# AsyncFlow-Sim/AsyncFlow

Measured on AMD Instinct MI355X. Metric: simulated request-events/sec (2-server LB scenario, 10k replicas/GPU), higher is better.
Workload: dtype f64

## Files before the change

### asyncflow_amd/csrc/af_core.hpp

```cpp
#pragma once

#include <stdint.h>

#include "af_math.hpp"

#if defined(__HIPCC__)
#define AF_CORE __device__ __forceinline__
#define AF_CORE_NOINLINE __device__ __noinline__
#define AF_PLAN_AS __attribute__((address_space(3)))
#else
#define AF_CORE inline
#define AF_CORE_NOINLINE __attribute__((noinline))
#define AF_PLAN_AS
#endif

namespace af {

enum : uint32_t { NODE_CLIENT = 0, NODE_LB = 1, NODE_SERVER = 2 };
enum : uint32_t { LB_ROUND_ROBIN = 0, LB_LEAST_CONNECTIONS = 1 };
enum : uint32_t { METRIC_READY = 1, METRIC_IO = 2, METRIC_RAM = 4, METRIC_EDGE = 8 };
enum : uint32_t {
    FLAG_POOL_OVERFLOW = 1u << 0,
    FLAG_FIFO_OVERFLOW = 1u << 1,
    FLAG_CLOCK_OVERFLOW = 1u << 2,
// ... 51 lines not shown
struct Layout {
    uint32_t cap;
    uint32_t fcap;
    uint32_t ovr_mask;
    uint32_t hk, ha, hb, edge, ring, stime, srv, cq, rq, lb, n_words;
    uint32_t srvram, marks;
    uint32_t tcap, tie_words;
};
#ifndef AF_RING_LOW
#define AF_RING_LOW 1
#endif
enum : uint32_t { LEDGE = 2, LSRV = 6, RING = 4, RING_LOW = AF_RING_LOW };

AF_HD Layout make_layout(uint32_t cap, uint32_t fcap, uint32_t n_edges, uint32_t n_servers, uint32_t n_lb,
                         uint32_t n_rows, uint32_t ovr_mask, uint32_t n_emarks = 0u, uint32_t n_smarks = 0u) {
    Layout L{};
    L.cap = cap;
    L.fcap = fcap;
    L.ovr_mask = ovr_mask;
    uint32_t w = 0;
    L.hk = w; w += cap;
    L.ha = w; w += cap;
    L.hb = w; w += cap;
    L.edge = w; w += LEDGE * n_edges;
    L.ring = w; w += RING * (1u + n_edges);
    L.stime = w; if (ovr_mask & (1u << PARAM_STEP_TIME)) w += n_rows;
    L.srv = w; w += LSRV * n_servers;
    L.cq = w; w += 2u * n_servers * fcap;
    L.rq = w; w += 2u * n_servers * fcap;
    L.lb = w; w += n_lb > 8u ? n_lb : 0u;
    L.srvram = w; if (ovr_mask & (1u << PARAM_SRV_RAM_MB)) w += n_servers;
    L.marks = w; if (ovr_mask & kParamMarkBits) w += 3u * n_emarks + 2u * n_smarks;
    L.n_words = w;
    uint32_t tc = 16u;
    while (tc < 2u * cap + 8u) tc <<= 1;
    L.tcap = tc;
    L.tie_words = 6u * tc + (2u + n_servers + 63u) / 64u + 17u;
    return L;
}
AF_HD uint64_t layout_bytes_per_lane(const Layout& L) { return 8ull * L.n_words; }

struct LaneOut {
    double* clock;
    uint32_t* samples;
    uint32_t* counts;
    uint32_t clock_cap, tick_cap, series_pitch;
    uint32_t* hist;
    uint32_t* rps;
    uint32_t hist_bins, rps_buckets;
    double hist_scale;
};

#if defined(__HIP_DEVICE_COMPILE__)
#define AF_BUMP(p) ((void)atomicAdd((p), 1u))
#else
#define AF_BUMP(p) ((void)(*(p) += 1u))
#endif

AF_HD void store4(uint32_t* p, uint32_t a, uint32_t b, uint32_t c, uint32_t d) {
#if defined(__HIP_DEVICE_COMPILE__)
    *reinterpret_cast<uint4*>(p) = make_uint4(a, b, c, d);
#else
    p[0] = a; p[1] = b; p[2] = c; p[3] = d;
#endif
}

constexpr double AF_INF = __builtin_huge_val();

struct PreDraws {
    const double* base;
    uint32_t n_per_stream;
    uint32_t flags_in;
    uint64_t* tie;
    AF_HD double entry(uint32_t stream, uint32_t index) const {
        return base[(size_t)stream * n_per_stream + index];
    }
};

AF_HD double pre_edge_draw(uint64_t seed, uint32_t e, uint32_t idx, uint32_t dist, double mean, double sigma,
                           double dropout) {
    const uint32_t stream = stream_edge(e);
    const U4 r = draw_block(seed, stream, idx, 0u);
    if (u53(r.x, r.y) < dropout) return -1.0;
    return test_quant(variate_from_u1(dist, mean, sigma, u53(r.z, r.w), seed, stream, idx));
}

struct GenState {
    double g_now = 0.0, g_wend = 0.0, g_lam = 0.0;
    uint32_t draws = 0;
};
AF_HD double gen_next_gap(GenState& g, uint64_t seed, uint32_t users_dist, double users_mean, double users_sigma,
                          double rpm, double window_s, double T) {
    const double rps_per_user = rpm / 60.0;
    while (g.g_now < T) {
        if (g.g_now >= g.g_wend) {
            g.g_wend = g.g_now + window_s;
            const uint32_t idx = g.draws++;
            double users;
            if (users_dist == DIST_NORMAL) {
                const double v = users_mean + users_sigma * af_norminv(uniform_j(seed, STREAM_GENERATOR, idx, 0u));
                users = v > 0.0 ? v : 0.0;
            } else {
                users = (double)af_poisson(users_mean, seed, STREAM_GENERATOR, idx, 0u);
            }
            g.g_lam = users * rps_per_user;
        }
        if (g.g_lam <= 0.0) {
            g.g_now = g.g_wend;
            continue;
        }
        const U4 r = draw_block(seed, STREAM_GENERATOR, g.draws++, 0u);
        double u = u53(r.x, r.y);
        if (u < 1e-15) u = 1e-15;
        const double dt = test_quant(-af_log_unit(1.0 - u) / g.g_lam);
        if (g.g_now + dt > T) break;
        if (g.g_now + dt >= g.g_wend) {
            g.g_now = g.g_wend;
            continue;
        }
        g.g_now += dt;
        return dt;
    }
    g.g_now = T + 1.0;
    return -1.0;
}

AF_CORE_NOINLINE uint32_t cold_endpoint_pick(uint64_t seed, uint32_t sv, uint32_t idx, uint32_t n_ep) {
    const U4 r = draw_block(seed, stream_server(sv), idx, 0u);
    return (uint32_t)(((uint64_t)r.x * n_ep) >> 32);
}

struct LaneRegs {
    double now, t_gen, t_tick, t_emark, t_smark;
    uint64_t lb_list;
    uint32_t q_gen, q_tick, q_emark, q_smark;
    uint32_t arr_ahead;
    int32_t dirty_edge;
    uint32_t fl;
    uint32_t heap_n, seq, live, max_live, lb_n, emark_i, smark_i;
    uint32_t n_gen, n_comp, n_drop, n_events, n_ticks, n_marks, flags;
    uint32_t pb_n;
};

template <bool kFaithful> struct RoundType { using type = uint32_t; };
template <> struct RoundType<false> { using type = bool; };

template <class Mem, bool kFaithful = true>
struct Lane : LaneRegs {
    const PlanView& P;
    const Layout& L;
    Mem M;
    LaneOut O;
    PreDraws D;
    uint64_t seed;

    enum : uint32_t {
        F_HOLE = 1u,
        F_GRANT = 2u,
        F_SEND = 4u,
        F_ADV = 8u,
        F_ADV_CORE = 16u,
        F_ADV_IO = 32u,
        F_DIRTY_ARR = 64u,
        F_SEND_FIRST = 128u
    };

    uint32_t pend_count;
// ... 1116 lines not shown
```

### asyncflow_amd/csrc/af_flow.hpp

```cpp
#pragma once

#include <stdint.h>

#include "af_core.hpp"

namespace aff {

using af::AF_INF;
using af::d2u;
using af::u2d;

enum : uint32_t {
    FLAG_FLOW_FALLBACK = 1u << 8,
    FLOW_WHY_TIE = 1u << 9,
    FLOW_WHY_LIST = 1u << 10,
    FLOW_WHY_RING = 1u << 11,
    FLOW_WHY_RAM = 1u << 12,
    FLOW_WHY_GEN_TIE = 1u << 15,
    FLOW_WHY_MASK = FLOW_WHY_TIE | FLOW_WHY_LIST | FLOW_WHY_RING | FLOW_WHY_RAM | FLOW_WHY_GEN_TIE,
};
constexpr uint32_t kMaxServers = 16;
constexpr uint32_t kSrvSlots = 16;
enum : uint32_t { LBW_ARRIVALS = 24u, LBW_SEG_OFF = LBW_ARRIVALS + kSrvSlots, LBW_SEG_LEN = LBW_SEG_OFF + kSrvSlots,
                  LBW_PROG = LBW_SEG_LEN + kSrvSlots, LBW_SLOTS = LBW_PROG + kSrvSlots, LBW_U32 = LBW_SLOTS + kSrvSlots };
// ... 365 lines not shown
                            if (u < n_left) {
                                if (!in_hbm) ring()[((r0 + u) & (R - 1u)) * pitch + ser] = 0;
                                value += d[u];
                                samples[(size_t)(r0 + u) * pitch + ser] = series_word(value, on, is_ram);
                            }
                    }
                }
            }
        }
        tick_base = upto;
    }

    AF_CORE double spike_at(uint32_t e, double now) {
        double sp = 0.0;
        if (A.n_edge_marks <= 32u) {
            for (uint32_t m = sends()[e]; m != 0u; m &= m - 1u) {
                const uint32_t i = (uint32_t)__builtin_ctz(m);
                const double tm = u2d(emark(i)[0]);
                if (tm < now) sp = spike_cum()[i];
                else if (tm == now) why |= FLOW_WHY_TIE;
            }
            return sp;
        }
        for (uint32_t i = 0u; i < A.n_edge_marks; ++i) {
            const double tm = u2d(emark(i)[0]);
            if ((uint32_t)emark(i)[2] != e) continue;
            if (tm < now) sp = spike_cum()[i];
            else if (tm == now) why |= FLOW_WHY_TIE;
        }
        return sp;
    }
    AF_CORE double send_floor(uint32_t st, double h, bool cached = true) {
        if (!(kMarks && A.n_edge_marks != 0u) || !(h < AF_INF)) return h;
        if (kLC && st == 2u) return h;
        AF_PLAN_AS double* c = fcache() + 3u * st;
        double until = c[0], sp_min = c[1], cand = c[2];
        if (!cached || !(h < until)) {
            until = cand = sp_min = AF_INF;
            const uint32_t n_out = st == 2u ? A.n_lb_edges : st == 3u ? A.n_servers : 1u;
            for (uint32_t k = 0u; k < n_out; ++k) {
                const uint32_t e = st == 0u   ? A.gen_out_edge
                                   : st == 1u ? A.client_out_edge
                                   : st == 2u ? (uint32_t)blob[A.off_lb + k]
                                              : (uint32_t)(blob[A.off_srv + af::SREC * k + 1u] >> 16) & 0xFFFFu;
                double sp = 0.0;
                for (uint32_t i = 0u; i < A.n_edge_marks; ++i) {
                    if ((uint32_t)emark(i)[2] != e) continue;
                    const double tm = u2d(emark(i)[0]), after = spike_cum()[i];
                    if (tm < h) {
                        sp = after;
                    } else {
                        until = tm < until ? tm : until;
                        cand = tm + after < cand ? tm + after : cand;
                    }
                }
                sp_min = sp < sp_min ? sp : sp_min;
            }
            if (cached && lane == 0u) {
                c[0] = until;
                c[1] = sp_min;
                c[2] = cand;
            }
        }
        const double fl = h + sp_min;
        return fl < cand ? fl : cand;
    }
    AF_CORE_NOINLINE static double cold_variate(uint32_t dist, double mean, double sigma, double u1, uint64_t seed, uint32_t stream,
                                                uint32_t idx) {
        return af::variate_from_u1(dist, mean, sigma, u1, seed, stream, idx);
    }
    AF_CORE bool edge_draw(uint32_t e, uint32_t idx, double& transit) const {
        const AF_PLAN_AS uint64_t* r = erec(e);
        const double mean = u2d(r[0]), sigma = u2d(r[1]);
        const uint32_t stream = af::stream_edge(e);
#if defined(__HIP_DEVICE_COMPILE__) && defined(AF_FJ_KEYS_PER_CALL)
        uint32_t sd_lo = (uint32_t)__builtin_amdgcn_readfirstlane((int)(uint32_t)seed), sd_hi = (uint32_t)__builtin_amdgcn_readfirstlane((int)(uint32_t)(seed >> 32));
        asm volatile("" : "+s"(sd_lo), "+s"(sd_hi));
        const af::U4 rr = af::draw_block(((uint64_t)sd_hi << 32) | sd_lo, stream, idx, 0u);
#else
        const af::U4 rr = af::draw_block(seed, stream, idx, 0u);
#endif
        const uint64_t k53 = ((uint64_t)(rr.x >> 5) << 26) | (uint64_t)(rr.y >> 6);
        const bool sent = !(k53 < r[2]);
        const double u1 = af::u53(rr.z, rr.w);
#if defined(AF_FJ_DIST_ALL) && (AF_FJ_DIST_ALL != 255)
        transit = af::test_quant(af::variate_from_u1(AF_FJ_DIST_ALL, mean, sigma, u1, seed, stream, idx));
#else
        const uint32_t dist = (uint32_t)(r[3] >> 16) & 0xFFu;
        transit = af::test_quant(dist == af::DIST_EXPONENTIAL ? -(mean * af::af_log_unit(1.0 - u1)) : cold_variate(dist, mean, sigma, u1, seed, stream, idx));
#endif
        return sent;
    }
    AF_CORE bool send_draw(uint32_t e, uint32_t idx, double& transit, bool pre = false, double pre_transit = 0.0) {
        transit = pre_transit;
        const bool sent = (kLC && pre) ? !(pre_transit < 0.0) : edge_draw(e, idx, transit);
        if (!sent) drops += 1u;
        return sent;
    }
    AF_CORE bool send_finish(uint32_t e, double now, uint32_t row_now, bool have_row, double transit, double& key, bool& counted) {
        counted = false;
        const double spike = (kMarks && A.n_edge_marks != 0u) ? spike_at(e, now) : 0.0;
        key = now + (transit + spike);
        if (transit + spike < 0.0) why |= FLOW_WHY_TIE;
        if (!kFar) {
            if (samples != nullptr) add_span(e, have_row ? row_now : tick_index(now, true), tick_index(key, true), 1);
        } else if (samples != nullptr) {
            const uint32_t ib = tick_index(key, true);
            if (ib != row_now) {
                add_point(e, row_now, 1);
                const uint32_t R = A.L.ring_rows, N = A.n_ticks < A.tick_cap ? A.n_ticks : A.tick_cap;
                if ((kHbmRing && R == 0u) || ib >= N || ib - tick_base < R) add_point(e, ib, -1);
                else counted = true;
            }
        }
        return true;
    }

    AF_CORE void append(uint32_t s, bool have, double key, double t0, uint32_t aux, double sent) {
        const uint64_t m = W::ballot(have);
        const uint32_t n = n_list_get(s);
        const uint32_t pos = n + W::mbcnt(m);
        if (have) {
            list_key(s)[pos] = key;
            list_t0(s)[pos] = t0;
            if (kTieBreak) list_ts(s)[pos] = sent;
            if (s == 2u || (kFar && s == 3u)) list_aux(s)[pos] = (uint16_t)aux;
        }
        n_list_set(s, n + popc64(m));
    }

    AF_CORE uint32_t select(uint32_t s, double H_in, uint32_t room, double& okey, double& ot0, uint32_t& oaux, uint32_t hs, uint32_t level = kAnyLevel) {
        if (kBig) return select_big(s, H_in, room, okey, ot0, oaux, hs, level);
        return select_regs<IPL>(s, H_in, room, okey, ot0, oaux, hs, level);
    }
    template <uint32_t IPLx>
    AF_CORE uint32_t select_regs(uint32_t s, double H_in, uint32_t room, double& okey, double& ot0, uint32_t& oaux, uint32_t hs, uint32_t level) {
        W::sync();
        const double lo = H_get(hs);
        const double hi_t = H_in < A.total_time ? H_in : A.total_time, hi = (kFar && t_lim < hi_t) ? t_lim : hi_t;
        const uint32_t n = n_list_get(s);
        okey = AF_INF;
        ot0 = 0.0;
        oaux = 0u;
        if (!(hi > lo)) return 0u;
        if (n == 0u) {
            H_set(hs, hi);
            return 0u;
        }
        AF_PLAN_AS double* K = list_key(s);
        AF_PLAN_AS double* T0 = list_t0(s);
        AF_PLAN_AS double* TS = list_ts(s);
        AF_PLAN_AS uint16_t* AX = list_aux(s);
        double sc = 64.0 * W::rcp(hi - lo);
        if (!(sc < 1e300)) sc = 1e300;
        hist()[lane] = 0u;
        W::sync();
        double k[IPLx], t[IPLx], sent[IPLx];
        uint32_t a[IPLx], b[IPLx], slot[IPLx];
        bool valid[IPLx], elig[IPLx];
#pragma unroll
        for (uint32_t q = 0u; q < IPLx; ++q) {
            valid[q] = elig[q] = false;
            k[q] = t[q] = sent[q] = 0.0;
            a[q] = b[q] = slot[q] = 0u;
            {
                const uint32_t i = q * 64u + lane;
                valid[q] = i < n;
                k[q] = K[i];
                t[q] = T0[i];
                if (kTieBreak) sent[q] = TS[i];
                a[q] = (s == 2u || (kFar && s == 3u)) ? AX[i] : 0u;
                elig[q] = valid[q] && k[q] < hi && (!kChain || level == kAnyLevel || level_of(a[q] & (kSrvSlots - 1u)) == level);
// ... 1813 lines not shown
```

### asyncflow_amd/csrc/af_math.hpp

```cpp
#pragma once

#include <stdint.h>

#if defined(__HIPCC__)
#define AF_HD __host__ __device__ __forceinline__
#else
#define AF_HD inline
#endif

namespace af {

constexpr uint32_t STREAM_GENERATOR = 0u;
AF_HD uint32_t stream_edge(uint32_t e) { return 1u + e; }
AF_HD uint32_t stream_server(uint32_t s) { return 0x1000u + s; }

struct U4 {
    uint32_t x, y, z, w;
};

AF_HD U4 philox4x32_10(uint32_t c0, uint32_t c1, uint32_t c2, uint32_t c3, uint32_t k0, uint32_t k1) {
#pragma unroll
    for (int r = 0; r < 10; ++r) {
        const uint64_t p0 = (uint64_t)0xD2511F53u * c0;
        const uint64_t p1 = (uint64_t)0xCD9E8D57u * c2;
        const uint32_t n0 = (uint32_t)(p1 >> 32) ^ c1 ^ k0;
        const uint32_t n1 = (uint32_t)p1;
        const uint32_t n2 = (uint32_t)(p0 >> 32) ^ c3 ^ k1;
        const uint32_t n3 = (uint32_t)p0;
        c0 = n0;
        c1 = n1;
        c2 = n2;
        c3 = n3;
        k0 += 0x9E3779B9u;
        k1 += 0xBB67AE85u;
    }
    return U4{c0, c1, c2, c3};
}

AF_HD double u53(uint32_t hi, uint32_t lo) {
    return ((double)(hi >> 5) * 67108864.0 + (double)(lo >> 6)) * (1.0 / 9007199254740992.0);
}

AF_HD U4 draw_block(uint64_t seed, uint32_t stream, uint32_t index, uint32_t sub) {
    return philox4x32_10(index, sub, stream, 0u, (uint32_t)seed, (uint32_t)(seed >> 32));
}

AF_HD double uniform_j(uint64_t seed, uint32_t stream, uint32_t index, uint32_t j) {
    const U4 r = draw_block(seed, stream, index, j >> 1);
    return (j & 1u) ? u53(r.z, r.w) : u53(r.x, r.y);
}

AF_HD uint64_t f64_bits(double x) { return __builtin_bit_cast(uint64_t, x); }
AF_HD double bits_f64(uint64_t u) { return __builtin_bit_cast(double, u); }

AF_HD double af_sqrt(double x) { return __builtin_sqrt(x); }

AF_HD double af_log(double x) {
    constexpr double ln2_hi = 6.93147180369123816490e-01, ln2_lo = 1.90821492927058770002e-10;
    constexpr double L1 = 6.666666666666735130e-01, L2 = 3.999999999940941908e-01,
                     L3 = 2.857142874366239149e-01, L4 = 2.222219843214978396e-01,
                     L5 = 1.818357216161805012e-01, L6 = 1.531383769920937332e-01,
                     L7 = 1.479819860511658591e-01;
    uint64_t u = f64_bits(x);
    uint32_t hx = (uint32_t)(u >> 32);
    int k = 0;
    if (hx < 0x00100000u || (hx >> 31)) {
        if ((u << 1) == 0) return -__builtin_inf();
        if (hx >> 31) return __builtin_nan("");
        k -= 54;
        x *= 18014398509481984.0;
        u = f64_bits(x);
        hx = (uint32_t)(u >> 32);
    } else if (hx >= 0x7ff00000u) {
        return x;
    } else if (hx == 0x3ff00000u && (u << 32) == 0) {
        return 0.0;
    }
    hx += 0x3ff00000u - 0x3fe6a09eu;
    k += (int)(hx >> 20) - 0x3ff;
    hx = (hx & 0x000fffffu) + 0x3fe6a09eu;
    x = bits_f64(((uint64_t)hx << 32) | (u & 0xffffffffull));

    const double f = x - 1.0;
    const double hfsq = 0.5 * f * f;
    const double s = f / (2.0 + f);
    const double z = s * s;
    const double w = z * z;
    const double t1 = w * (L2 + w * (L4 + w * L6));
    const double t2 = z * (L1 + w * (L3 + w * (L5 + w * L7)));
    const double R = t2 + t1;
    const double dk = (double)k;
    return s * (hfsq + R) + dk * ln2_lo - hfsq + f + dk * ln2_hi;
}

AF_HD double af_log_unit(double x) {
    constexpr double ln2_hi = 6.93147180369123816490e-01, ln2_lo = 1.90821492927058770002e-10;
    constexpr double L1 = 6.666666666666735130e-01, L2 = 3.999999999940941908e-01,
                     L3 = 2.857142874366239149e-01, L4 = 2.222219843214978396e-01,
                     L5 = 1.818357216161805012e-01, L6 = 1.531383769920937332e-01,
                     L7 = 1.479819860511658591e-01;
    const uint64_t u = f64_bits(x);
    uint32_t hx = (uint32_t)(u >> 32);
    hx += 0x3ff00000u - 0x3fe6a09eu;
    const int k = (int)(hx >> 20) - 0x3ff;
    hx = (hx & 0x000fffffu) + 0x3fe6a09eu;
    x = bits_f64(((uint64_t)hx << 32) | (u & 0xffffffffull));
    const double f = x - 1.0;
    const double hfsq = 0.5 * f * f;
    const double s = f / (2.0 + f);
    const double z = s * s;
    const double w = z * z;
    const double t1 = w * (L2 + w * (L4 + w * L6));
    const double t2 = z * (L1 + w * (L3 + w * (L5 + w * L7)));
    const double R = t2 + t1;
    const double dk = (double)k;
    return s * (hfsq + R) + dk * ln2_lo - hfsq + f + dk * ln2_hi;
}

AF_HD double af_exp(double x) {
    constexpr double ln2hi = 6.93147180369123816490e-01, ln2lo = 1.90821492927058770002e-10,
                     invln2 = 1.44269504088896338700e+00;
    constexpr double P1 = 1.66666666666666019037e-01, P2 = -2.77777777770155933842e-03,
                     P3 = 6.61375632143793436117e-05, P4 = -1.65339022054652515390e-06,
                     P5 = 4.13813679705723846039e-08;
    if (x != x) return x;
    if (x > 709.782712893383973096) return __builtin_inf();
    if (x < -745.13321910194110842) return 0.0;
    const double ax = x < 0 ? -x : x;
    double hi, lo;
    int k;
    if (ax > 0.34657359027997264) {
        if (ax >= 1.0397207708399179) {
            k = (int)(invln2 * x + (x < 0 ? -0.5 : 0.5));
        } else {
            k = x < 0 ? -1 : 1;
        }
        hi = x - (double)k * ln2hi;
        lo = (double)k * ln2lo;
        x = hi - lo;
    } else if (ax > 3.725290298461914e-09) {
        k = 0;
        hi = x;
        lo = 0.0;
    } else {
        return 1.0 + x;
    }
    const double xx = x * x;
    const double c = x - xx * (P1 + xx * (P2 + xx * (P3 + xx * (P4 + xx * P5))));
    const double y = 1.0 + (x * c / (2.0 - c) - lo + hi);
    if (k == 0) return y;
    const int k1 = k / 2, k2 = k - k1;
    const double f1 = bits_f64((uint64_t)(0x3ff + k1) << 52);
    const double f2 = bits_f64((uint64_t)(0x3ff + k2) << 52);
    return y * f1 * f2;
}

AF_HD double af_norminv(double p) {
    const double q = p - 0.5;
    double r, val;
    if ((q < 0 ? -q : q) <= 0.425) {
        r = 0.180625 - q * q;
        return q *
               (((((((r * 2509.0809287301226727 + 33430.575583588128105) * r + 67265.770927008700853) * r +
                    45921.953931549871457) * r + 13731.693765509461125) * r + 1971.5909503065514427) * r +
                 133.14166789178437745) * r + 3.387132872796366608) /
               (((((((r * 5226.495278852545925 + 28729.085735721942674) * r + 39307.89580009271061) * r +
                    21213.794301586595867) * r + 5394.1960214247511077) * r + 687.1870074920579083) * r +
                 42.313330701600911252) * r + 1.0);
    }
    r = q < 0 ? p : 1.0 - p;
    if (r <= 0.0) return q < 0 ? -__builtin_inf() : __builtin_inf();
    r = af_sqrt(-af_log(r));
    if (r <= 5.0) {
        r -= 1.6;
        val = (((((((r * 7.7454501427834140764e-4 + 0.0227238449892691845833) * r + 0.24178072517745061177) * r +
                   1.27045825245236838258) * r + 3.64784832476320460504) * r + 5.7694972214606914055) * r +
                4.6303378461565452959) * r + 1.42343711074968357734) /
              (((((((r * 1.05075007164441684324e-9 + 5.475938084995344946e-4) * r + 0.0151986665636164571966) * r +
                   0.14810397642748007459) * r + 0.68976733498510000455) * r + 1.6763848301838038494) * r +
                2.05319162663775882187) * r + 1.0);
    } else {
        r -= 5.0;
        val = (((((((r * 2.01033439929228813265e-7 + 2.71155556874348757815e-5) * r + 0.0012426609473880784386) * r +
                   0.026532189526576123093) * r + 0.29656057182850489123) * r + 1.7848265399172913358) * r +
                5.4637849111641143699) * r + 6.6579046435011037772) /
              (((((((r * 2.04426310338993978564e-15 + 1.4215117583164458887e-7) * r + 1.8463183175100546818e-5) * r +
                   7.868691311456132591e-4) * r + 0.0148753612908506148525) * r + 0.13692988092273580531) * r +
                0.59983220655588793769) * r + 1.0);
    }
    return q < 0 ? -val : val;
}

// ... 56 lines not shown
```

### asyncflow_amd/csrc/af_pregen.hpp

```cpp
#pragma once

#include <stdint.h>

#include "af_core.hpp"

namespace afp {

constexpr uint32_t kBatch = 8u;
constexpr uint32_t kRound = 8u;
constexpr uint32_t kChunk = kBatch * kRound;

AF_HD double unit_variate(uint64_t seed, uint32_t idx) {
    const af::U4 r = af::draw_block(seed, af::STREAM_GENERATOR, idx, 0u);
    double u = af::u53(r.x, r.y);
    if (u < 1e-15) u = 1e-15;
    return -af::af_log_unit(1.0 - u);
}

AF_HD double refine_rcp(double d, double r0) {
    const double e0 = __builtin_fma(-d, r0, 1.0);
    const double r1 = __builtin_fma(r0, e0, r0);
    const double e1 = __builtin_fma(-d, r1, 1.0);
    return __builtin_fma(r1, e1, r1);
}
AF_HD double div_by(double n, double d, double r2) {
    const double q = n * r2;
    const double rem = __builtin_fma(-d, q, n);
    return __builtin_fma(rem, r2, q);
}
AF_HD bool div_in_range(double d) { return d >= 0x1p-64 && d <= 0x1p64; }
AF_HD double rcp_estimate(double d) {
#if defined(__HIP_DEVICE_COMPILE__)
    return __builtin_amdgcn_rcp(d);
#else
    return (double)(1.0f / (float)d);
#endif
}

enum : uint32_t { LANE_WAIT = 0u, LANE_RUN = 1u, LANE_DONE = 2u };
constexpr uint32_t kFlagDrawOverflow = 1u << 6;

struct Lane {
    double g_now, g_wend, lam, rinv, t;
    uint32_t draws, k, flags, state;
    bool fast_div;
};
AF_HD void lane_init(Lane& L) {
    L.g_now = L.g_wend = L.lam = L.rinv = L.t = 0.0;
    L.draws = L.k = L.flags = 0u;
    L.state = LANE_WAIT;
    L.fast_div = false;
}
template <class UsersDraw>
AF_HD void window_start(Lane& L, double T, double window_s, double rps_per_user, UsersDraw&& users) {
    if (!(L.g_now < T)) {
        L.state = LANE_DONE;
        return;
    }
    L.g_wend = L.g_now + window_s;
    L.lam = users(L.draws++) * rps_per_user;
    if (L.lam <= 0.0) {
        L.g_now = L.g_wend;
        return;
    }
    L.fast_div = div_in_range(L.lam);
    L.rinv = L.fast_div ? refine_rcp(L.lam, rcp_estimate(L.lam)) : 0.0;
    L.state = LANE_RUN;
}
template <bool FAST_DIV>
AF_HD void lane_sums(const Lane& L, const double (&e)[kBatch], double (&G)[kBatch], double (&S)[kBatch]) {
    double g = L.g_now, s = L.t;
#pragma unroll
    for (uint32_t j = 0u; j < kBatch; ++j) {
        const double dt = af::test_quant(FAST_DIV ? div_by(e[j], L.lam, L.rinv) : e[j] / L.lam);
        g += dt;
        s = s + dt;
        G[j] = g;
        S[j] = s;
    }
}
AF_HD bool lane_usual(const Lane& L, const double (&G)[kBatch], double T, uint32_t n_draw) {
    return (G[kBatch - 1u] <= T) & (G[kBatch - 1u] < L.g_wend) & (L.k + kBatch <= n_draw);
}
AF_HD void lane_commit(Lane& L, const double (&G)[kBatch], const double (&S)[kBatch]) {
    L.k += kBatch;
    L.draws += kBatch;
    L.g_now = G[kBatch - 1u];
    L.t = S[kBatch - 1u];
}
AF_HD void lane_slow(Lane& L, const double (&G)[kBatch], const double (&S)[kBatch], double T, uint32_t n_draw, double* out,
                     bool stored) {
    uint32_t first = kBatch;
    bool over = false;
#pragma unroll
    for (uint32_t j = 0u; j < kBatch; ++j)
        if (first == kBatch && (G[j] > T || G[j] >= L.g_wend)) {
            first = j;
            over = G[j] > T;
        }
    uint32_t n_acc = first;
    bool full = false;
    if (L.k + n_acc > n_draw) {
        n_acc = n_draw - L.k;
        full = true;
    }
    if (!stored) {
        double* o = out + L.k;
#pragma unroll
        for (uint32_t j = 0u; j < kBatch; ++j)
            if (j < n_acc) o[j] = S[j];
    }
    L.k += n_acc;
    if (full) {
        L.flags = kFlagDrawOverflow;
        L.state = LANE_DONE;
    } else if (first == kBatch) {
        L.g_now = G[kBatch - 1u];
        L.t = S[kBatch - 1u];
        L.draws += kBatch;
    } else {
#pragma unroll
        for (uint32_t j = 0u; j + 1u < kBatch; ++j)
            if (j + 1u == first) L.t = S[j];
        L.draws += first + 1u;
        if (over) {
            L.state = LANE_DONE;
        } else {
            L.g_now = L.g_wend;
            L.state = LANE_WAIT;
        }
    }
}
template <bool FAST_DIV>
AF_HD void lane_step(Lane& L, const double (&e)[kBatch], double T, uint32_t n_draw, double* out) {
    double G[kBatch], S[kBatch];
    lane_sums<FAST_DIV>(L, e, G, S);
    if (lane_usual(L, G, T, n_draw)) {
        double* o = out + L.k;
#pragma unroll
        for (uint32_t j = 0u; j < kBatch; ++j) o[j] = S[j];
        lane_commit(L, G, S);
    } else {
        lane_slow(L, G, S, T, n_draw, out, false);
    }
}

AF_HD double users_draw(uint32_t dist, double mean, double sigma, uint64_t seed, uint32_t idx) {
    if (dist == af::DIST_NORMAL) {
        const double v = mean + sigma * af::af_norminv(af::uniform_j(seed, af::STREAM_GENERATOR, idx, 0u));
// ... 177 lines not shown
```

### asyncflow_amd/csrc/engine.hip

```cpp
#include <hip/hip_runtime.h>
#include <dlfcn.h>

#include <algorithm>
#include <chrono>
#include <cmath>
#include <cstdio>
#include <cstring>
#include <functional>
#include <string>
#include <vector>

#include "../../include/asyncflow_hip.h"
#include "af_core.hpp"
#include "af_flow_host.hpp"
#include "af_plan_pack.hpp"
#include "af_pregen.hpp"
#include "af_summary.hpp"
#include "af_pooled.hpp"
#include "af_series_windows.hpp"
#include "af_series_quantiles.hpp"
#include "af_series_excursions.hpp"
#include "af_series_histogram.hpp"
#include "af_series_combined.hpp"
#include "af_series_joint.hpp"
// ... 601 lines not shown
        g.out = a.draws;
        g.pre_flags = a.pre_flags;
        if (hipFuncSetAttribute(reinterpret_cast<const void*>(afp::af_arrival_groups), hipFuncAttributeMaxDynamicSharedMemorySize,
                                (int)sizeof(afp::GroupLds)) != hipSuccess)
            return 1;
        hipLaunchKernelGGL(afp::af_arrival_groups, dim3((n + g.group - 1u) / g.group), dim3(afp::kGroupThreads),
                           sizeof(afp::GroupLds), stream, g);
        return 0;
    }
    double best = 1e300;
    uint32_t best_s = 4u;
    for (uint32_t s : {4u, 5u, 8u}) {
        const double waves = std::ceil((double)n / (double)s);
        if (s != 4u && (!uniform_load || waves / 1024.0 < 1.9)) continue;
        const double cost = std::ceil(waves / 1024.0) * (4.06 * (double)s + 8.0);
        if (cost < best - 1e-9) {
            best = cost;
            best_s = s;
        }
    }
    bool rows = true;
    if (const char* env = std::getenv("AF_PREGEN_SCEN_PER_WAVE")) {
        const uint32_t v = (uint32_t)std::atoi(env);
        if (v == 4u || v == 5u || v == 8u) {
            best_s = v;
            rows = false;
        }
    }
    if (rows) {
        hipLaunchKernelGGL(af_pregen_arrivals_rows, dim3((n + 3u) / 4u), dim3(64), 0, stream, a, stride);
        return 0;
    }
    const dim3 grid((n + best_s - 1u) / best_s);
    if (best_s == 4u) hipLaunchKernelGGL(af_pregen_arrivals<16>, grid, dim3(64), 0, stream, a, stride);
    else if (best_s == 5u) hipLaunchKernelGGL(af_pregen_arrivals<12>, grid, dim3(64), 0, stream, a, stride);
    else hipLaunchKernelGGL(af_pregen_arrivals<8>, grid, dim3(64), 0, stream, a, stride);
    return 0;
}

__global__ void af_zero_online(const KArgs a, uint32_t count) {
    const uint32_t j = blockIdx.x;
    if (j >= count) return;
    const uint32_t sc = a.scen_map[j];
    if (a.online_hist)
        for (uint32_t i = threadIdx.x; i < a.online_hist_bins; i += blockDim.x) a.online_hist[(size_t)sc * a.online_hist_bins + i] = 0u;
    if (a.online_rps)
        for (uint32_t i = threadIdx.x; i < a.online_rps_buckets; i += blockDim.x) a.online_rps[(size_t)sc * a.online_rps_buckets + i] = 0u;
}

__global__ void __launch_bounds__(256) af_pregen_edges(const KArgs a) {
    const uint32_t i = blockIdx.x * blockDim.x + threadIdx.x;
    if (i >= a.n_draw) return;
    const uint32_t slot = blockIdx.y;
    const uint32_t scen = a.scen_map ? a.scen_map[slot] : slot;
    const uint32_t e = blockIdx.z;
    const uint64_t* rec = reinterpret_cast<const uint64_t*>(a.blob) + a.off_edge + af::EREC * e;
    const double mean = ovr_or(a, af::PARAM_EDGE_MEAN, e, scen, af::u2d(rec[0]));
    const double sigma = ovr_or(a, af::PARAM_EDGE_SIGMA, e, scen, af::u2d(rec[1]));
    const double dropout = ovr_or(a, af::PARAM_EDGE_DROPOUT, e, scen, af::u2d(rec[2]));
    const uint32_t dist = (uint32_t)(rec[3] >> 16) & 0xFFu;
    a.draws[((size_t)slot * (1u + a.n_edges) + 1u + e) * a.n_draw + i] =
        af::pre_edge_draw(a.seeds[scen], e, i, dist, mean, sigma, dropout);
}

__global__ void af_probe_kernel(int kind, uint64_t seed, const double* in, const double* in2, double* out, size_t n) {
    const size_t i = (size_t)blockIdx.x * blockDim.x + threadIdx.x;
    if (i >= n) return;
    const double x = in[i];
    const double y = in2 ? in2[i] : 0.0;
    double r;
    switch (kind) {
        case 0: {
            const uint32_t packed = (uint32_t)y;
            r = af::uniform_j(seed, packed >> 16, (uint32_t)x, packed & 0xFFFFu);
            break;
        }
        case 1: r = af::af_log(x); break;
        case 2: r = af::af_exp(x); break;
        case 3: r = af::af_norminv(x); break;
        case 4: r = af::af_sqrt(x); break;
        case 5: r = x / y; break;
        case 6: r = (double)af::af_poisson(x, seed, (uint32_t)y >> 16, (uint32_t)y & 0xFFFFu, 0u); break;
        case 7: r = af::af_log_unit(x); break;
        default: r = 0.0;
    }
    out[i] = r;
}

__global__ void __launch_bounds__(64) af_probe_store_wide(uint32_t* out, size_t words_per_wave) {
    uint32_t* base = out + (size_t)blockIdx.x * words_per_wave;
    for (size_t w = (size_t)threadIdx.x * 4u; w + 4u <= words_per_wave; w += 256u) af::store4(base + w, 1u, 2u, 3u, 4u);
}
__global__ void __launch_bounds__(64) af_probe_store_pairs16(uint32_t* out, size_t words_per_wave, uint32_t lanes) {
    uint32_t* base = out + (size_t)blockIdx.x * words_per_wave;
    for (size_t w0 = 0; w0 + 4u * lanes <= words_per_wave; w0 += 4u * lanes)
        if (threadIdx.x < lanes) af::store4(base + w0 + 4u * threadIdx.x, 1u, 2u, 3u, 4u);
}
__global__ void __launch_bounds__(64) af_probe_store_rows48(uint32_t* out, size_t words_per_wave) {
    uint32_t* base = out + (size_t)blockIdx.x * words_per_wave;
    for (size_t w0 = 0; w0 + 60u <= words_per_wave; w0 += 60u)
        if (threadIdx.x < 60u) base[w0 + threadIdx.x] = (uint32_t)w0;
}

thread_local std::string g_err;

int fail(int code, const std::string& msg) {
    g_err = msg;
    return code;
}

#define HIP_TRY(expr)                                                                              \
    do {                                                                                           \
        hipError_t e_ = (expr);                                                                    \
        if (e_ != hipSuccess)                                                                      \
            return fail(AF_ERR_HIP, std::string(#expr) + ": " + hipGetErrorString(e_));            \
    } while (0)

uint32_t pow2_at_least(uint32_t v) {
    uint32_t p = 1;
    while (p < v) p <<= 1;
    return p;
}

}

template <bool kLds, bool kFaithful, int WPE>
const void* des_kernel_klog(uint32_t klog) {
    switch (klog) {
        case 0: return reinterpret_cast<const void*>(af_des_kernel<kLds, kFaithful, 0, WPE>);
        case 1: return reinterpret_cast<const void*>(af_des_kernel<kLds, kFaithful, 1, WPE>);
        case 2: return reinterpret_cast<const void*>(af_des_kernel<kLds, kFaithful, 2, WPE>);
        case 3: return reinterpret_cast<const void*>(af_des_kernel<kLds, kFaithful, 3, WPE>);
        case 4: return reinterpret_cast<const void*>(af_des_kernel<kLds, kFaithful, 4, WPE>);
        case 5: return reinterpret_cast<const void*>(af_des_kernel<kLds, kFaithful, 5, WPE>);
        default: return reinterpret_cast<const void*>(af_des_kernel<kLds, kFaithful, 6, WPE>);
    }
}
const void* des_kernel_for(bool lds, bool faithful, uint32_t klog, bool roomy) {
    if (!faithful) return lds ? des_kernel_klog<true, false, 3>(klog) : des_kernel_klog<false, false, 3>(klog);
    if (roomy) return lds ? des_kernel_klog<true, true, 2>(klog) : des_kernel_klog<false, true, 2>(klog);
    return lds ? des_kernel_klog<true, true, 3>(klog) : des_kernel_klog<false, true, 3>(klog);
}

struct af_engine {
    int device = 0;
    bool plan_only = false;
    hipStream_t stream = nullptr;
    hipEvent_t ev0 = nullptr, ev1 = nullptr, ev2 = nullptr;
    KArgs args{};
    unsigned char* d_blob = nullptr;
    unsigned char* d_state = nullptr;
    size_t state_cap = 0;
    void* d_sweep = nullptr;
    size_t sweep_cap = 0;
    double* d_draws = nullptr;
    size_t draws_cap = 0;
    uint32_t* d_pre_flags = nullptr;
    size_t pre_flags_cap = 0;
    uint64_t* d_tie = nullptr;
    size_t tie_cap = 0;
    uint32_t* d_n_shared = nullptr;
    uint32_t* d_map = nullptr;
    size_t map_cap = 0;
    uint32_t* d_order = nullptr;
    size_t order_cap = 0;
    const af_summary_t* fused_sum = nullptr;
// ... 3384 lines not shown
```

Measured before the change: 123.4 billion.

## Streamline RNG draw arithmetic with bitop3 XOR, FMA u53, and rcp-based log division

The Philox rounds now use a three-input XOR builtin where available. The 53-bit uniform is built with an FMA, and 1-u is computed as a single FMA from the integer key. The division inside af_log_unit is replaced by a hardware reciprocal estimate with Newton refinement and a correction step. Together these aim to cut ALU work in the hot per-event random-variate path, at the risk of small rounding differences versus the old exact division and subtraction. Probe cases for draw_block and one_minus_unit_of are added to the math probe kernel.

```diff
diff --git a/asyncflow_amd/csrc/af_core.hpp b/asyncflow_amd/csrc/af_core.hpp
--- a/asyncflow_amd/csrc/af_core.hpp
+++ b/asyncflow_amd/csrc/af_core.hpp
@@ -157,7 +157,9 @@
     const uint32_t stream = stream_edge(e);
     const U4 r = draw_block(seed, stream, idx, 0u);
     if (u53(r.x, r.y) < dropout) return -1.0;
-    return test_quant(variate_from_u1(dist, mean, sigma, u53(r.z, r.w), seed, stream, idx));
+    const double K1 = k53(r.z, r.w);
+    return test_quant(dist == DIST_EXPONENTIAL ? -(mean * af_log_unit(one_minus_unit_of(K1)))
+                                               : variate_from_u1(dist, mean, sigma, unit_of(K1), seed, stream, idx));
 }
 
 struct GenState {
diff --git a/asyncflow_amd/csrc/af_flow.hpp b/asyncflow_amd/csrc/af_flow.hpp
--- a/asyncflow_amd/csrc/af_flow.hpp
+++ b/asyncflow_amd/csrc/af_flow.hpp
@@ -471,12 +471,14 @@
 #endif
         const uint64_t k53 = ((uint64_t)(rr.x >> 5) << 26) | (uint64_t)(rr.y >> 6);
         const bool sent = !(k53 < r[2]);
-        const double u1 = af::u53(rr.z, rr.w);
+        const double K1 = af::k53(rr.z, rr.w);
 #if defined(AF_FJ_DIST_ALL) && (AF_FJ_DIST_ALL != 255)
-        transit = af::test_quant(af::variate_from_u1(AF_FJ_DIST_ALL, mean, sigma, u1, seed, stream, idx));
+        transit = af::test_quant(AF_FJ_DIST_ALL == af::DIST_EXPONENTIAL ? -(mean * af::af_log_unit(af::one_minus_unit_of(K1)))
+                                                                        : af::variate_from_u1(AF_FJ_DIST_ALL, mean, sigma, af::unit_of(K1), seed, stream, idx));
 #else
         const uint32_t dist = (uint32_t)(r[3] >> 16) & 0xFFu;
-        transit = af::test_quant(dist == af::DIST_EXPONENTIAL ? -(mean * af::af_log_unit(1.0 - u1)) : cold_variate(dist, mean, sigma, u1, seed, stream, idx));
+        transit = af::test_quant(dist == af::DIST_EXPONENTIAL ? -(mean * af::af_log_unit(af::one_minus_unit_of(K1)))
+                                                              : cold_variate(dist, mean, sigma, af::unit_of(K1), seed, stream, idx));
 #endif
         return sent;
     }
diff --git a/asyncflow_amd/csrc/af_math.hpp b/asyncflow_amd/csrc/af_math.hpp
--- a/asyncflow_amd/csrc/af_math.hpp
+++ b/asyncflow_amd/csrc/af_math.hpp
@@ -17,15 +17,37 @@
 struct U4 {
     uint32_t x, y, z, w;
 };
+
+#if !defined(AF_DRAW_BITOP3)
+#define AF_DRAW_BITOP3 1
+#endif
+#if !defined(AF_DRAW_UNSCALED_DIV)
+#define AF_DRAW_UNSCALED_DIV 1
+#endif
+#if !defined(AF_DRAW_FMA_U53)
+#define AF_DRAW_FMA_U53 1
+#endif
+
+AF_HD uint32_t xor3(uint32_t a, uint32_t b, uint32_t c) {
+#if defined(__HIP_DEVICE_COMPILE__) && AF_DRAW_BITOP3
+#if __has_builtin(__builtin_amdgcn_bitop3_b32)
+    return __builtin_amdgcn_bitop3_b32(a, b, c, 0x96u);
+#else
+    return a ^ b ^ c;
+#endif
+#else
+    return a ^ b ^ c;
+#endif
+}
 
 AF_HD U4 philox4x32_10(uint32_t c0, uint32_t c1, uint32_t c2, uint32_t c3, uint32_t k0, uint32_t k1) {
 #pragma unroll
     for (int r = 0; r < 10; ++r) {
         const uint64_t p0 = (uint64_t)0xD2511F53u * c0;
         const uint64_t p1 = (uint64_t)0xCD9E8D57u * c2;
-        const uint32_t n0 = (uint32_t)(p1 >> 32) ^ c1 ^ k0;
+        const uint32_t n0 = xor3((uint32_t)(p1 >> 32), c1, k0);
         const uint32_t n1 = (uint32_t)p1;
-        const uint32_t n2 = (uint32_t)(p0 >> 32) ^ c3 ^ k1;
+        const uint32_t n2 = xor3((uint32_t)(p0 >> 32), c3, k1);
         const uint32_t n3 = (uint32_t)p0;
         c0 = n0;
         c1 = n1;
@@ -37,9 +59,22 @@
     return U4{c0, c1, c2, c3};
 }
 
-AF_HD double u53(uint32_t hi, uint32_t lo) {
-    return ((double)(hi >> 5) * 67108864.0 + (double)(lo >> 6)) * (1.0 / 9007199254740992.0);
-}
+AF_HD double k53(uint32_t hi, uint32_t lo) {
+#if defined(__HIP_DEVICE_COMPILE__) && AF_DRAW_FMA_U53
+    return __builtin_fma((double)(hi >> 5), 67108864.0, (double)(lo >> 6));
+#else
+    return (double)(hi >> 5) * 67108864.0 + (double)(lo >> 6);
+#endif
+}
+AF_HD double unit_of(double K) { return K * (1.0 / 9007199254740992.0); }
+AF_HD double one_minus_unit_of(double K) {
+#if defined(__HIP_DEVICE_COMPILE__) && AF_DRAW_FMA_U53
+    return __builtin_fma(K, -(1.0 / 9007199254740992.0), 1.0);
+#else
+    return 1.0 - unit_of(K);
+#endif
+}
+AF_HD double u53(uint32_t hi, uint32_t lo) { return unit_of(k53(hi, lo)); }
 
 AF_HD U4 draw_block(uint64_t seed, uint32_t stream, uint32_t index, uint32_t sub) {
     return philox4x32_10(index, sub, stream, 0u, (uint32_t)seed, (uint32_t)(seed >> 32));
@@ -54,6 +89,13 @@
 AF_HD double bits_f64(uint64_t u) { return __builtin_bit_cast(double, u); }
 
 AF_HD double af_sqrt(double x) { return __builtin_sqrt(x); }
+
+AF_HD double refine_rcp(double d, double r0) {
+    const double e0 = __builtin_fma(-d, r0, 1.0);
+    const double r1 = __builtin_fma(r0, e0, r0);
+    const double e1 = __builtin_fma(-d, r1, 1.0);
+    return __builtin_fma(r1, e1, r1);
+}
 
 AF_HD double af_log(double x) {
     constexpr double ln2_hi = 6.93147180369123816490e-01, ln2_lo = 1.90821492927058770002e-10;
@@ -107,7 +149,14 @@
     x = bits_f64(((uint64_t)hx << 32) | (u & 0xffffffffull));
     const double f = x - 1.0;
     const double hfsq = 0.5 * f * f;
+#if defined(__HIP_DEVICE_COMPILE__) && AF_DRAW_UNSCALED_DIV
+    const double d = 2.0 + f;
+    const double r = refine_rcp(d, __builtin_amdgcn_rcp(d));
+    const double q = f * r;
+    const double s = __builtin_fma(__builtin_fma(-d, q, f), r, q);
+#else
     const double s = f / (2.0 + f);
+#endif
     const double z = s * s;
     const double w = z * z;
     const double t1 = w * (L2 + w * (L4 + w * L6));
diff --git a/asyncflow_amd/csrc/af_pregen.hpp b/asyncflow_amd/csrc/af_pregen.hpp
--- a/asyncflow_amd/csrc/af_pregen.hpp
+++ b/asyncflow_amd/csrc/af_pregen.hpp
@@ -12,17 +12,11 @@
 
 AF_HD double unit_variate(uint64_t seed, uint32_t idx) {
     const af::U4 r = af::draw_block(seed, af::STREAM_GENERATOR, idx, 0u);
-    double u = af::u53(r.x, r.y);
-    if (u < 1e-15) u = 1e-15;
-    return -af::af_log_unit(1.0 - u);
-}
-
-AF_HD double refine_rcp(double d, double r0) {
-    const double e0 = __builtin_fma(-d, r0, 1.0);
-    const double r1 = __builtin_fma(r0, e0, r0);
-    const double e1 = __builtin_fma(-d, r1, 1.0);
-    return __builtin_fma(r1, e1, r1);
-}
+    const double K = af::k53(r.x, r.y);
+    const double x = K < 1e-15 * 9007199254740992.0 ? 1.0 - 1e-15 : af::one_minus_unit_of(K);
+    return -af::af_log_unit(x);
+}
+
 AF_HD double div_by(double n, double d, double r2) {
     const double q = n * r2;
     const double rem = __builtin_fma(-d, q, n);
@@ -64,7 +58,7 @@
         return;
     }
     L.fast_div = div_in_range(L.lam);
-    L.rinv = L.fast_div ? refine_rcp(L.lam, rcp_estimate(L.lam)) : 0.0;
+    L.rinv = L.fast_div ? af::refine_rcp(L.lam, rcp_estimate(L.lam)) : 0.0;
     L.state = LANE_RUN;
 }
 template <bool FAST_DIV>
diff --git a/asyncflow_amd/csrc/engine.hip b/asyncflow_amd/csrc/engine.hip
--- a/asyncflow_amd/csrc/engine.hip
+++ b/asyncflow_amd/csrc/engine.hip
@@ -707,6 +707,14 @@
         case 5: r = x / y; break;
         case 6: r = (double)af::af_poisson(x, seed, (uint32_t)y >> 16, (uint32_t)y & 0xFFFFu, 0u); break;
         case 7: r = af::af_log_unit(x); break;
+        case 8:
+        case 9: {
+            const uint64_t sd = af::d2u(x), si = af::d2u(y);
+            const af::U4 b = af::draw_block(sd, (uint32_t)(si >> 32), (uint32_t)si, 0u);
+            r = af::u2d(kind == 8 ? ((uint64_t)b.x << 32) | b.y : ((uint64_t)b.z << 32) | b.w);
+            break;
+        }
+        case 10: r = af::one_minus_unit_of(af::k53((uint32_t)(af::d2u(x) >> 32), (uint32_t)af::d2u(x))); break;
         default: r = 0.0;
     }
     out[i] = r;
```

New measurement: 126.4 billion, median of 6. 1.02x the previous value.
